# cvjena/ITAL

Hardware: AMD Instinct MI355X
Metric: MI-scored candidates/sec per fetch_unlabelled(k) round (higher is better)
Workload: dtype f64; 1 GPU; USPS-shaped synthetic 9298x256, k=4, perfect user, full 2^t enumeration, fetch_unlabelled + update per step; n=9298, d=256, k=4, parallelism=candidate rows sharded over 1 GPU(s), 1 record all-gather per greedy step

## Files before the change

ital_amd/_lib.py:

```python
import ctypes
import os

HERE = os.path.dirname(os.path.abspath(__file__))
LIB_PATH = os.environ.get("ITAL_HIP_LIB", os.path.join(HERE, "libital_hip.so"))

c_void_p, c_int, c_int64, c_double = ctypes.c_void_p, ctypes.c_int, ctypes.c_int64, ctypes.c_double

ITAL_MAX_T = 8
ITAL_REC_HEADER = 10
ITAL_JUMP_BITS = 48
ITAL_GENERIC_MAX_DIM = 20
ITAL_GENERIC_MAX_REL = 16
ITAL_GENERIC_MAX_CALLS = 1 << 22
ITAL_TOPK_MAX = 4096
ITAL_ROUND_MAX_CAND = 1 << 21


class ItalBatch(ctypes.Structure):
    _fields_ = [("kmax", c_int), ("ldx", c_int), ("ldw", c_int), ("bidx", c_void_p), ("bgpos", c_void_p),
                ("bsort", c_void_p), ("bmu", c_void_p), ("sig", c_void_p), ("XB", c_void_p), ("XBn", c_void_p),
                ("VB", c_void_p)]


class ItalLabelBatch(ctypes.Structure):
# ... 113 lines not shown
    "ital_score_generic_join": (c_int, [c_void_p]),
    "ital_ctx_create": (c_int, [c_int64, c_int, c_double, c_double, c_double, c_int, c_int, c_int, c_void_p, c_void_p]),
    "ital_ctx_destroy": (c_int, [c_void_p]),
    "ital_ctx_fit": (c_int, [c_void_p, c_void_p, c_int, c_void_p]),
    "ital_ctx_update": (c_int, [c_void_p, c_void_p, c_void_p, c_int, c_void_p]),
    "ital_ctx_fetch": (c_int, [c_void_p, c_int, c_void_p, c_void_p]),
    "ital_ctx_predict_stored": (c_int, [c_void_p, c_void_p, c_void_p, c_void_p]),
    "ital_ctx_local_rows": (c_int64, [c_void_p, c_void_p]),
    "ital_record_len": (c_int, [c_int, c_int, c_int]),
    "ital_round_workspace": (c_int64, [c_int, c_int64, c_int64]),
    "ital_sel_parts_len": (c_int64, [c_int, c_int64, c_int64]),
    "ital_mcmi_round": (c_int, [ctypes.POINTER(ItalMcmiRoundDesc), c_void_p]),
    "ital_gather_block": (c_int, [c_void_p, c_int64, c_int64, c_int64, c_void_p, c_void_p, c_int, c_void_p, c_int64, c_int,
                                  c_void_p, c_void_p, c_void_p, c_void_p, c_int64, c_void_p, c_void_p, c_void_p, c_void_p]),
    "ital_select_resolve": (c_int, [c_void_p, c_int, c_int, c_int, c_int, c_int, ItalBatch, c_void_p, c_void_p,
                                    c_void_p]),
}


class ItalCtxModel(ctypes.Structure):
    _fields_ = [("label_prob", c_double), ("mistake_prob", c_double), ("label_estimation", c_int),
                ("monte_carlo_num_rel", c_int), ("monte_carlo_num_fb", c_int), ("clip_cov", c_double)]


CTX_SIGNATURES = {
    "ital_ctx_set_model": (c_int, [c_void_p, ctypes.POINTER(ItalCtxModel)]),
    "ital_ctx_fetch_list": (c_int, [c_void_p, c_int, c_void_p, c_int64, c_void_p, c_int, c_void_p, c_void_p]),
    "ital_ctx_mcmi_fetch": (c_int, [c_void_p, c_int, c_void_p, c_int64, c_void_p, c_void_p]),
    "ital_ctx_top_results": (c_int, [c_void_p, c_int, c_void_p, c_void_p]),
    "ital_ctx_predict": (c_int, [c_void_p, c_void_p, c_int64, c_void_p, c_void_p, c_void_p]),
}


DENSE_SIGNATURES = {
    "ital_gram_rows": (c_int, [c_void_p, c_void_p, c_int, c_void_p, c_void_p, c_void_p, c_void_p, c_int, c_int, c_double,
                               c_double, c_double, c_void_p]),
    "ital_chol_batched": (c_int, [c_void_p, c_void_p, c_void_p, c_int, c_int, c_void_p, c_void_p, c_void_p]),
    "ital_chol_solve_batched": (c_int, [c_void_p, c_void_p, c_void_p, c_void_p, c_int, c_void_p, c_void_p]),
    "ital_kernel_matvec": (c_int, [c_void_p, c_void_p, c_int64, c_void_p, c_void_p, c_int64, c_int, c_void_p, c_int64, c_int,
                                   c_double, c_double, c_void_p, c_int64, c_void_p, c_int64, c_void_p]),
    "ital_kernel_matvec_workspace": (c_int64, [c_int64, c_int64]),
}


ADAPT_SIGNATURES = {
    "ital_chol_inv_diag": (c_int, [c_void_p, c_int, c_int64, c_void_p, c_void_p, c_int64, c_void_p, c_void_p]),
    "ital_chol_inv_diag_workspace": (c_int64, [c_int]),
    "ital_adapt_scores": (c_int, [c_void_p, c_void_p, c_void_p, c_int64, c_double, c_void_p, c_void_p, c_void_p]),
    "ital_adapt_error": (c_int, [c_void_p, c_int64, c_void_p, c_int, c_int64, c_void_p, c_void_p, c_double, c_void_p,
                                 c_void_p, c_void_p]),
}


class ItalHipError(RuntimeError):
    pass


def load(path=LIB_PATH):
    if not os.path.exists(path):
        raise ImportError(
            f"{path} not found: build it with `python -m ital_amd.build` (hipcc, gfx950). "
            "ital_amd has no CPU fallback.")
    try:
        import torch
    except ImportError:
        pass
    lib = ctypes.CDLL(path)
    for name, (res, args) in list(SIGNATURES.items()) + list(CTX_SIGNATURES.items()) + list(DENSE_SIGNATURES.items()) + \
            list(ADAPT_SIGNATURES.items()):
        fn = getattr(lib, name)
        fn.restype = res
        fn.argtypes = args
    return lib


_lib = None


def lib():
    global _lib
    if _lib is None:
        _lib = load()
    return _lib


def check(rc):
    if rc != 0:
        raise ItalHipError(f"libital_hip: error {rc}: {lib().ital_last_error().decode()}")


def legacy_normals(n_skip, n_out, threads=1):
    import numpy as np
    n_skip, n_out = int(n_skip), int(n_out)
    state = np.random.get_state(legacy=True)
    if state[0] != "MT19937":
        if n_skip:
            np.random.standard_normal(n_skip)
        return np.random.standard_normal(n_out)
    st = ItalNpLegacyState()
    key = np.ascontiguousarray(state[1], dtype=np.uint32)
    ctypes.memmove(st.key, key.ctypes.data, 624 * 4)
    st.pos, st.has_gauss, st.gauss = int(state[2]), int(state[3]), float(state[4])
    out = np.empty(n_out, dtype=np.float64)
    check(lib().ital_np_legacy_normals(ctypes.byref(st), n_skip, out.ctypes.data, n_out, int(threads)))
    np.random.set_state(("MT19937", np.frombuffer(st.key, dtype=np.uint32).copy(), int(st.pos), int(st.has_gauss),
                         float(st.gauss)))
    return out
```

ital_amd/build.py:

```python
import os
import subprocess
import sys
from concurrent.futures import ThreadPoolExecutor

HERE = os.path.dirname(os.path.abspath(__file__))
CSRC = os.path.join(HERE, "csrc")
INCLUDE = os.path.join(os.path.dirname(HERE), "include")
LIB = os.path.join(HERE, "libital_hip.so")
SOURCES = ["api.hip", "rbf.hip", "chol.hip", "score.hip", "select.hip", "mcmi.hip", "score_generic.hip", "gen_pipeline.hip", "topk.hip", "exchange.hip", "round.hip", "ctx.hip", "dense.hip", "adapt.hip",
           "mvn_stream.cpp", "np_legacy.cpp"]
HIPCC = os.environ.get("HIPCC", "/opt/rocm/bin/hipcc")
EXTRA = os.environ.get("ITAL_HIPCC_EXTRA", "").split()
HOST_EXTRA = os.environ.get("ITAL_HOST_EXTRA", "").split()
LINK_EXTRA = os.environ.get("ITAL_LINK_EXTRA", "").split()
LIB = os.environ.get("ITAL_HIP_LIB_OUT", LIB)
FLAGS = EXTRA + ["--offload-arch=gfx950", "-O3", "-std=c++17", "-fPIC", "-fno-gpu-rdc",
         "-I", INCLUDE, "-I", CSRC, "-Wall", "-Wno-unused-function"]
HOST_FLAGS = ["-O3", "-std=c++17", "-fPIC", "-ffp-contract=off", "-I", INCLUDE, "-I", CSRC, "-Wall"]


def _newer(target, deps):
    if not os.path.exists(target):
        return True
    t = os.path.getmtime(target)
    return any(os.path.getmtime(d) > t for d in deps)


def build(force=False, verbose=False):
    headers = [os.path.join(CSRC, f) for f in os.listdir(CSRC) if f.endswith(".h")] + \
              [os.path.join(INCLUDE, "ital_hip.h"), os.path.join(INCLUDE, "ital_ctx.h"), os.path.join(INCLUDE, "ital_dense.h"),
               os.path.join(INCLUDE, "ital_adapt.h")]
    objdir = os.environ.get("ITAL_OBJ_DIR", os.path.join(HERE, "_obj"))
    os.makedirs(objdir, exist_ok=True)
    jobs = []
    objs = []
    for src in SOURCES:
        s = os.path.join(CSRC, src)
        o = os.path.join(objdir, os.path.splitext(src)[0] + ".o")
        objs.append(o)
        if force or _newer(o, [s] + headers):
            jobs.append([HIPCC] + (FLAGS if src.endswith(".hip") else HOST_FLAGS + HOST_EXTRA) + ["-c", s, "-o", o])

    def run(cmd):
        if verbose:
            print(" ".join(cmd), flush=True)
        subprocess.check_call(cmd)

    if jobs:
        with ThreadPoolExecutor(max_workers=4) as ex:
            list(ex.map(run, jobs))
    if jobs or force or _newer(LIB, objs):
        run([HIPCC, "--offload-arch=gfx950", "-shared", "-fPIC", "-o", LIB] + LINK_EXTRA + objs + ["-ldl", "-lpthread"])
    return LIB


if __name__ == "__main__":
    print(build(force="--force" in sys.argv, verbose=True))
```

ital_amd/csrc/score.hip:

```cpp
#include <hip/hip_runtime.h>
#include <stdint.h>

#include <type_traits>

#include "device_math.h"
#include "ital_hip.h"
#include "ital_internal.h"
#include "qmc_common.h"
#include "qmc_exact.h"
#include "qmc_seed.h"
#include "qmc_share.h"
#include "select_common.h"

#ifndef ITAL_QMC_HOTK
#define ITAL_QMC_HOTK 1
#endif
#ifndef ITAL_QMC_MAIN_NH
#define ITAL_QMC_MAIN_NH(T) ((T) == 6 || (T) == 8 ? 2 : 3)
#endif
#ifndef ITAL_QMC_WAVES
#define ITAL_QMC_WAVES(T) ((T) <= 4 || (T) == 6 || (T) == 8 ? 4 : 3)
#endif
#ifndef ITAL_QMC_MAIN_PS
#define ITAL_QMC_MAIN_PS(T) ((T) >= 7)
#endif
#ifndef ITAL_QMC_MAIN_KE6
#define ITAL_QMC_MAIN_KE6(T) ((T) == 8)
#endif
#ifndef ITAL_QMC_MAIN_KEN
#define ITAL_QMC_MAIN_KEN(T) ((T) == 7 ? 2 : -1)
#endif
#ifndef ITAL_QMC_MAIN_KE
#define ITAL_QMC_MAIN_KE(T) 1
#endif
#ifndef ITAL_QMC_MAIN_KS
#define ITAL_QMC_MAIN_KS(T) 0
#endif
#ifndef ITAL_QMC_MAIN_CFL
#define ITAL_QMC_MAIN_CFL(T) ((T) >= 7)
#endif

#ifndef ITAL_QMC_SHARE_LAST
#define ITAL_QMC_SHARE_LAST 1
#endif
#ifndef ITAL_QMC_SHARE_RECS
#define ITAL_QMC_SHARE_RECS 4
#endif
#ifndef ITAL_QMC_SHARE_VCF
#define ITAL_QMC_SHARE_VCF 3
#endif

namespace ital {

struct ScoreArgs {
    int t;
    int64_t n_cand;
    const int32_t* cand;
    const uint8_t* alive;
    const double* mu;
    const double* s2;
    const double* C;
    int64_t ldc;
    int64_t row_offset;
    int64_t pos_offset;
    const int64_t* gpos;
    ital_batch b;
    double noise, eps;
    int label_mode;
    double* mi;
    int seed[6];
    const long long* jump;
    const long long* jumppat;
    const double* vk;
    int* status;
    SelectTail sel;
};

__device__ __forceinline__ double log_eps(double p, double eps) { return log(p + eps); }

__device__ __forceinline__ void mi_accumulate(double& mi, double pr, double pu, double eps, int mode) {
    double cur = log_eps(pu, eps) - log_eps(pr, eps);
    if (mode == 1) {
        if (cur > mi) mi = cur;
    } else if (mode == 2) {
        if (mi == 0 || cur < mi) mi = cur;
    } else {
        mi += cur * pr;
    }
}

__global__ __launch_bounds__(256) void score_t1_kernel(ScoreArgs a) {
    const int64_t p = (int64_t)blockIdx.x * blockDim.x + threadIdx.x;
    const bool valid = p < a.n_cand && a.alive[p];
    double mi = 0.0;
    if (valid) {
        const int row = a.cand[p];
        const double mu = a.mu[row];
        const double su = a.s2[row];
        const double sc = fmax(0.0, su);
        const double p_irr = norm_cdf0(mu, sqrt(sc));
        const double w = 1.0 / (su + a.noise);
        const double g = su * w;
// ... 43 lines not shown
            const double c00 = a.noise * g00, c11 = a.noise * g11, c01 = a.noise * g01;
            const double t0 = sqrt(c00), t1 = sqrt(c11);
            double h = -u0 / t0, k = -u1 / t1;
            const double rho = c01 / (t0 * t1);
            const int64_t gi = a.row_offset + row;
            if (gi < a.b.bidx[0]) val = bvn_orthant(k, h, rel1, rel0, rho);
            else val = bvn_orthant(h, k, rel0, rel1, rho);
        }
    }
    vals[updated ? 1 : 0][pair] = val;
    __syncthreads();
    Best c = {0.0, -1, 0};
    if (threadIdx.x < 32) {
        const int64_t pc = (int64_t)blockIdx.x * 32 + threadIdx.x;
        if (pc < a.n_cand && a.alive[pc]) {
            double mi = 0.0;
#pragma unroll
            for (int q = 0; q < 4; q++) mi_accumulate(mi, vals[0][4 * threadIdx.x + q], vals[1][4 * threadIdx.x + q], a.eps, a.label_mode);
            a.mi[pc] = mi;
            c.val = mi;
            c.pos = a.gpos ? a.gpos[pc] : a.pos_offset + pc;
            c.loc = pc;
        }
    }
    if (a.sel.enabled) {
        c = block_best(c, 0);
        select_tail(a.sel, c, blockIdx.x, gridDim.x, true, gridDim.x);
    }
}

template <int T>
struct Qmc {
    static constexpr int NDIM = T - 1;
    static constexpr int NP = NDIM < 10 ? NDIM : 10;
    static constexpr int PRIME = P_TAB[NP - 1];
    static constexpr int NCOV = T * (T + 1) / 2;
    static constexpr int NCOR = T * (T - 1) / 2;
    static constexpr int NPAT = 1 << T;
    static constexpr int NCALLS = 2 << T;
    static constexpr int LAT = 8 * NDIM * 2;
    static constexpr int LATP = 5 * NDIM;
    static constexpr int R_LIM = NCOR, R_META = NCOR + T, R_LAT = NCOR + T + 1;
    static constexpr int REC = R_LAT + LATP;
    static constexpr int SLAB_RAW = NCOV + 2 * T + NDIM;
    static constexpr int SLAB = SLAB_RAW | 1;
    static constexpr int PREP_THREADS = T <= 6 ? 256 : 128;
    static constexpr int NH = ITAL_QMC_MAIN_NH(T);
    static constexpr int TAILQ = 128 * NH;
    static constexpr bool PS = ITAL_QMC_MAIN_PS(T), CFL = PS && ITAL_QMC_MAIN_CFL(T);
    static constexpr bool SHARE = ITAL_QMC_SHARE_LAST && ITAL_QMC_HOTK && ITAL_QMC_FLIP && !PS &&
                                  QmcRounds<T, NH>::NCL == 1 && ITAL_QMC_SHARE_RECS * QmcRounds<T, NH>::REST <= 64 &&
                                  NPAT % ITAL_QMC_SHARE_RECS == 0;
    static constexpr int RPW = SHARE ? ITAL_QMC_SHARE_RECS : 1;
    static constexpr int WAVE_DOUBLES = LAT + TAILQ + (CFL ? NCOR + T : 0) + (SHARE ? 64 + 2 * RPW + 6 : 0);
    typedef typename std::conditional<(CFL && ITAL_QMC_MAIN_KS(T)), HotKS,
                typename std::conditional<(ITAL_QMC_MAIN_KEN(T) >= 0), HotKEn<(ITAL_QMC_MAIN_KEN(T) >= 0 ? ITAL_QMC_MAIN_KEN(T) : 0)>,
                typename std::conditional<(ITAL_QMC_MAIN_KE6(T)), HotKE6,
                    typename std::conditional<(ITAL_QMC_MAIN_KE(T)), HotKE, HotK>::type>::type>::type>::type Coef;
    static constexpr int64_t CAND_DOUBLES = (int64_t)NPAT * (REC + 1) + 3;
};
constexpr long long META_EVAL = 1, META_PRIOR_ONE = 2, META_POST_ONE = 4;
constexpr long long META_EXACT = 8;

template <int T>
__device__ void rcswp(int p, int q, double* cov, double* lim, unsigned& infi) {
    double tmp = lim[p]; lim[p] = lim[q]; lim[q] = tmp;
    unsigned bp = (infi >> p) & 1u, bq = (infi >> q) & 1u;
    infi = (infi & ~((1u << p) | (1u << q))) | (bq << p) | (bp << q);
    tmp = cov[pidx(p, p)]; cov[pidx(p, p)] = cov[pidx(q, q)]; cov[pidx(q, q)] = tmp;
    for (int j = 0; j < p; j++) { tmp = cov[pidx(p, j)]; cov[pidx(p, j)] = cov[pidx(q, j)]; cov[pidx(q, j)] = tmp; }
    for (int i = p + 1; i < q; i++) { tmp = cov[pidx(i, p)]; cov[pidx(i, p)] = cov[pidx(q, i)]; cov[pidx(q, i)] = tmp; }
    for (int i = q + 1; i < T; i++) { tmp = cov[pidx(i, p)]; cov[pidx(i, p)] = cov[pidx(i, q)]; cov[pidx(i, q)] = tmp; }
}

template <int T>
__device__ bool covsrt(double* cov, double* lim, double* y, unsigned& infi) {
    const double SQTWPI = 2.506628274631001, EPS = 1e-10;
    bool ok = true;
    for (int i = 0; i < T; i++) {
        double dmin = 0, emin = 1, zmin = 0, cvdiag = 0;
        int jmin = i;
        for (int j = i; j < T; j++) {
            const double cjj = cov[pidx(j, j)];
            if (cjj > EPS) {
                const double sumsq = sqrt_pos(cjj);
                double sum = 0;
                for (int k = 0; k < i; k++) sum += cov[pidx(j, k)] * y[k];
                const double z = fast_div(lim[j] - sum, sumsq);
                const double ph = mvn_phi(z);
                const bool lower = (infi >> j) & 1u;
                const double d = lower ? ph : 0.0;
                const double e = lower ? 1.0 : fmax(ph, 0.0);
                if (emin + d >= e + dmin) { jmin = j; zmin = z; dmin = d; emin = e; cvdiag = sumsq; }
            }
        }
        if (jmin > i) rcswp<T>(i, jmin, cov, lim, infi);
        cov[pidx(i, i)] = cvdiag;
        if (cvdiag > 0) {
            const double rdiag = fast_div(1.0, cvdiag);
            for (int l = i + 1; l < T; l++) {
                cov[pidx(l, i)] = cov[pidx(l, i)] * rdiag;
                for (int j = i + 1; j <= l; j++) cov[pidx(l, j)] -= cov[pidx(l, i)] * cov[pidx(j, i)];
            }
            const bool lower = (infi >> i) & 1u;
            if (emin > dmin + EPS) {
                const double dens = -exp_neg(-zmin * zmin / 2) * (1.0 / SQTWPI);
                const double yl = lower ? dens : 0.0, yu = lower ? 0.0 : dens;
// ... 134 lines not shown
            atomicOr(a.status, 2);
        } else {
            bool sat1 = true, sat0 = false;
            for (int v = 0; v < T; v++) {
                double bound = 0;
                for (int j = 0; j < v; j++) bound += fabs(cov[pidx(v, j)]) * 9.0;
                const bool lower = (infi >> v) & 1u;
                if (lower) {
                    if (!(lim[v] + bound < -37.0)) sat1 = false;
                    if (lim[v] - bound > 37.0) sat0 = true;
                } else {
                    if (!(lim[v] - bound > 37.0)) sat1 = false;
                    if (lim[v] + bound < -37.0) sat0 = true;
                }
            }
            if (sat0) verdict = 4;
            else if (sat1) verdict = 2;
            else evaluate = true;
        }
    }
    if (verdict == 2) meta |= META_PRIOR_ONE;
    if (evaluate) {
        meta |= META_EVAL | ((long long)infi << 8);
        const unsigned fl = ITAL_QMC_FLIP ? infi : 0u;
        for (int v = 1; v < T; v++)
            for (int j = 0; j < v; j++)
                rec[v * (v - 1) / 2 + j] = (((fl >> v) ^ (fl >> j)) & 1u) ? -cov[pidx(v, j)] : cov[pidx(v, j)];
        for (int v = 0; v < T; v++) rec[Q::R_LIM + v] = ((fl >> v) & 1u) ? -lim[v] : lim[v];
        const int* sp = seeds + i * 6;
        MrgState sti = {sp[0], sp[1], sp[2], sp[3], sp[4], sp[5]};
        mrg_apply(sti, a.jumppat + (int64_t)r * 18);
        MrgStateF st = mrg_to_f(sti);
        for (int j = 0; j < Q::NDIM; j++) gen[j] = (double)j;
        unsigned int* shifts = reinterpret_cast<unsigned int*>(rec + Q::R_LAT);
        unsigned char* perm = reinterpret_cast<unsigned char*>(rec + Q::R_LAT + 4 * Q::NDIM);
        for (int sft = 0; sft < 8; sft++) {
            for (int j = 1; j <= Q::NDIM - 1; j++) {
                const double u = mrg_next_f(st);
                const int jp = (int)(j + u * (Q::NDIM + 1 - j));
                const double xt = gen[j - 1];
                gen[j - 1] = gen[jp - 1];
                gen[jp - 1] = xt;
            }
            for (int j = 0; j < Q::NDIM; j++) perm[sft * Q::NDIM + j] = (unsigned char)gen[j];
            for (int j = 0; j < Q::NDIM; j++) shifts[sft * Q::NDIM + j] = (unsigned int)mrg_next_z(st);
        }
    }
    rec[Q::R_META] = __longlong_as_double(meta);
}

template <int T>
__device__ __forceinline__ void qmc_main_shared(const uint8_t* __restrict__ alive, int64_t slab_lo, int64_t slab_n,
                                                const double* __restrict__ recs, const double* __restrict__ vk, double eps,
                                                int label_mode, double* __restrict__ terms) {
    using Q = Qmc<T>;
    using R = QmcRounds<T, Q::NH>;
    extern __shared__ double lds_all[];
    const int lane = threadIdx.x & 63;
    const int wid = __builtin_amdgcn_readfirstlane(threadIdx.x >> 6);
    const int64_t item0 = ((int64_t)blockIdx.x * 4 + wid) * Q::RPW;
    const int64_t i = item0 >> T;
    if (i >= slab_n) return;
    if (!alive[slab_lo + i]) return;
    double* lat = lds_all + (size_t)wid * Q::WAVE_DOUBLES;
    double* tailq = lat + Q::LAT;
    int first = -1;
    for (int j = Q::RPW - 1; j >= 0; j--)
        if (__double_as_longlong(uniform_f64(recs[(item0 + j) * Q::REC + Q::R_META])) & META_EVAL) first = j;
    double* lastv = tailq + Q::TAILQ;
    typename Q::Coef kk;
    kk.load();
    if (first >= 0) {
        const int j_own = lane >> 4;
        bool dead = j_own >= Q::RPW;
        if (!dead) dead = !(__double_as_longlong(recs[(item0 + j_own) * Q::REC + Q::R_META]) & META_EVAL);
        const double* rec = recs + (item0 + (dead ? first : j_own)) * Q::REC;
        const unsigned flips = (unsigned)(__double_as_longlong(rec[Q::R_META]) >> 8) & ((1u << T) - 1u);
        double cf[Q::NCOR > 0 ? Q::NCOR : 1], lm[T], xx[Q::NDIM > 0 ? Q::NDIM : 1];
#pragma unroll
        for (int q = 0; q < Q::NCOR; q++) cf[q] = rec[q];
#pragma unroll
        for (int q = 0; q < T; q++) lm[q] = rec[Q::R_LIM + q];
        const unsigned int* shifts = reinterpret_cast<const unsigned int*>(rec + Q::R_LAT);
        const unsigned char* perm = reinterpret_cast<const unsigned char*>(rec + Q::R_LAT + 4 * Q::NDIM);
        const int it = R::FULL * 64 * Q::NH + ((lane & 15) >> 1);
        const int sft = it / Q::PRIME;
        const int k = it - sft * Q::PRIME + 1;
#pragma unroll
        for (int j = 0; j < Q::NDIM; j++) {
            const int q = sft * Q::NDIM + j;
            const double gen = vk[perm[q]];
            const double shf = (double)shifts[q] * MRG_INVMP1 + (((flips >> (q % Q::NDIM)) & 1u) ? 0.5 : 0.0);
            const double v = k * gen + shf;
            const double fr = v - floor(v);
            const double x = fabs(2 * fr - 1);
            xx[j] = (lane & 1) ? 1 - x : x;
        }
        double w0;
        lastv[lane] = eval_chain_lanes<T, typename Q::Coef>(xx, dead, cf, lm, flips, tailq, lane, kk, w0);
        if ((lane & 15) == 0 && j_own < Q::RPW) lastv[64 + Q::RPW + j_own] = w0;
    }
    double* keep = lastv + 64 + 2 * Q::RPW;
    if (lane == 0) {
        keep[0] = __longlong_as_double((long long)recs);
        keep[1] = __longlong_as_double((long long)vk);
        keep[2] = __longlong_as_double((long long)terms);
        keep[3] = eps;
        keep[4] = __longlong_as_double((long long)label_mode);
        keep[5] = __longlong_as_double(item0);
    }
    __builtin_amdgcn_fence(__ATOMIC_RELEASE, "wavefront");
    __builtin_amdgcn_wave_barrier();
    __builtin_amdgcn_fence(__ATOMIC_ACQUIRE, "wavefront");
    int jv = 0;
    for (;;) {
        int ln = lane;
        __asm__ volatile("" : "+v"(ln), "+v"(jv));
        const int j = __builtin_amdgcn_readfirstlane(jv);
        if (j >= Q::RPW) break;
        const double* rec = reinterpret_cast<const double*>(__double_as_longlong(uniform_f64(keep[0]))) +
                            (__double_as_longlong(uniform_f64(keep[5])) + j) * Q::REC;
        const long long meta = __double_as_longlong(uniform_f64(rec[Q::R_META]));
        double pr = (meta & META_PRIOR_ONE) ? 1.0 : 0.0;
        if (meta & META_EVAL) {
            const unsigned flips = (unsigned)(meta >> 8) & ((1u << T) - 1u);
            __builtin_amdgcn_fence(__ATOMIC_RELEASE, "wavefront");
            __builtin_amdgcn_wave_barrier();
            {
                const double* vk_j = reinterpret_cast<const double*>(__double_as_longlong(uniform_f64(keep[1])));
                const unsigned int* shifts = reinterpret_cast<const unsigned int*>(rec + Q::R_LAT);
                const unsigned char* perm = reinterpret_cast<const unsigned char*>(rec + Q::R_LAT + 4 * Q::NDIM);
                for (int q = ln; q < 8 * Q::NDIM; q += 64) {
                    lat[q] = vk_j[perm[q]];
                    lat[8 * Q::NDIM + q] = (double)shifts[q] * MRG_INVMP1 + (((flips >> (q % Q::NDIM)) & 1u) ? 0.5 : 0.0);
                }
            }
            double cf[Q::NCOR > 0 ? Q::NCOR : 1], lm[T];
#pragma unroll
            for (int q = 0; q < Q::NCOR; q++) cf[q] = q >= Q::NCOR - ITAL_QMC_SHARE_VCF ? rec[q] : uniform_f64(rec[q]);
#pragma unroll
            for (int q = 0; q < T; q++) lm[q] = uniform_f64(rec[Q::R_LIM + q]);
            __builtin_amdgcn_fence(__ATOMIC_RELEASE, "wavefront");
            __builtin_amdgcn_wave_barrier();
            __builtin_amdgcn_fence(__ATOMIC_ACQUIRE, "wavefront");
            const double w0 = lastv[64 + Q::RPW + j];
            const double part = qmc_lane_sum_full<T, typename Q::Coef, Q::NH>(lat, w0, cf, lm, flips, tailq, ln, kk);
            __asm__ volatile("" : "+v"(jv));
            const int j2 = __builtin_amdgcn_readfirstlane(jv);
            const double acc = part + (ln < 16 ? lastv[16 * j2 + ln] : 0.0);
            pr = wave_sum(acc) / (16.0 * Q::PRIME);
#ifndef ITAL_NO_EXACT_FLAG
            if ((pr > 1.0 - EXACT_BAND || pr < EXACT_BAND) && ln == 0 && __double_as_longlong(keep[4]) != 0) {
                double* rm = reinterpret_cast<double*>(__double_as_longlong(keep[0])) + (__double_as_longlong(keep[5]) + j2) * Q::REC + Q::R_META;
                *rm = __longlong_as_double(__double_as_longlong(*rm) | META_EXACT);
            }
#endif
        }
        __asm__ volatile("" : "+v"(jv));
        if (ln == 0) lastv[64 + __builtin_amdgcn_readfirstlane(jv)] = pr;
        jv = jv + 1;
    }
    __builtin_amdgcn_fence(__ATOMIC_RELEASE, "wavefront");
    __builtin_amdgcn_wave_barrier();
    __builtin_amdgcn_fence(__ATOMIC_ACQUIRE, "wavefront");
    if (lane < Q::RPW) {
        const double* recs_k = reinterpret_cast<const double*>(__double_as_longlong(keep[0]));
        double* terms_k = reinterpret_cast<double*>(__double_as_longlong(keep[2]));
        const long long item_l = __double_as_longlong(keep[5]) + lane;
        const double eps_k = keep[3];
        const double pr_l = lastv[64 + lane];
        const long long meta_l = __double_as_longlong(recs_k[item_l * Q::REC + Q::R_META]);
        const double pu = (meta_l & META_POST_ONE) ? 1.0 : 0.0;
        const double cur = log_eps(pu, eps_k) - log_eps(pr_l, eps_k);
        terms_k[item_l] = __double_as_longlong(keep[4]) == 0 ? cur * pr_l : cur;
    }
}

template <int T>
__global__ __launch_bounds__(256) __attribute__((amdgpu_waves_per_eu(ITAL_QMC_WAVES(T), ITAL_QMC_WAVES(T)))) void qmc_main_kernel(
    const uint8_t* __restrict__ alive, int64_t slab_lo, int64_t slab_n, const double* __restrict__ recs,
    const double* __restrict__ vk, double eps, int label_mode, double* __restrict__ terms) {
    using Q = Qmc<T>;
    if constexpr (Q::SHARE) {
        qmc_main_shared<T>(alive, slab_lo, slab_n, recs, vk, eps, label_mode, terms);
        return;
    }
    extern __shared__ double lds_all[];
    const int lane = threadIdx.x & 63;
    const int wid = __builtin_amdgcn_readfirstlane(threadIdx.x >> 6);
    const int64_t item = (int64_t)blockIdx.x * 4 + wid;
    const int64_t i = item >> T;
    if (i >= slab_n) return;
    if (!alive[slab_lo + i]) return;
    const double* rec = recs + item * Q::REC;
    const long long meta = __double_as_longlong(uniform_f64(rec[Q::R_META]));
    double pr = (meta & META_PRIOR_ONE) ? 1.0 : 0.0;
    if (meta & META_EVAL) {
        double* lat = lds_all + (size_t)wid * Q::WAVE_DOUBLES;
        double* tailq = lat + Q::LAT;
        const unsigned flips = ITAL_QMC_FLIP ? (unsigned)(meta >> 8) & ((1u << T) - 1u) : 0u;
        {
            const unsigned int* shifts = reinterpret_cast<const unsigned int*>(rec + Q::R_LAT);
            const unsigned char* perm = reinterpret_cast<const unsigned char*>(rec + Q::R_LAT + 4 * Q::NDIM);
            for (int q = lane; q < 8 * Q::NDIM; q += 64) {
                lat[q] = vk[perm[q]];
                lat[8 * Q::NDIM + q] = (double)shifts[q] * MRG_INVMP1 + (((flips >> (q % Q::NDIM)) & 1u) ? 0.5 : 0.0);
            }
        }
        double cf[Q::NCOR > 0 ? Q::NCOR : 1], lm[T];
        double* slab = tailq + Q::TAILQ;
        if (Q::CFL) {
            for (int q = lane; q < Q::NCOR + T; q += 64) slab[q] = rec[q];
        } else {
#pragma unroll
            for (int q = 0; q < Q::NCOR; q++) cf[q] = uniform_f64(rec[q]);
#pragma unroll
            for (int q = 0; q < T; q++) lm[q] = uniform_f64(rec[Q::R_LIM + q]);
        }
        const unsigned infi = (unsigned)(meta >> 8) & ((1u << T) - 1u);
        __builtin_amdgcn_fence(__ATOMIC_RELEASE, "wavefront");
        __builtin_amdgcn_wave_barrier();
        __builtin_amdgcn_fence(__ATOMIC_ACQUIRE, "wavefront");
#if ITAL_QMC_HOTK
        typename Q::Coef kk;
        kk.load();
        constexpr bool FL = ITAL_QMC_FLIP != 0;
        const double acc = Q::PS ? qmc_lane_sum_ps<T, typename Q::Coef, Q::NH, Q::CFL, FL>(lat, cf, lm, slab, infi, tailq, lane, kk)
                                 : qmc_lane_sum<T, typename Q::Coef, Q::NH, FL>(lat, cf, lm, infi, tailq, lane, kk);
#else
        const double acc = qmc_lane_sum<T, LitK, Q::NH, ITAL_QMC_FLIP != 0>(lat, cf, lm, infi, tailq, lane);
#endif
        pr = wave_sum(acc) / (16.0 * Q::PRIME);
#ifndef ITAL_NO_EXACT_FLAG
        if (label_mode != 0 && (pr > 1.0 - EXACT_BAND || pr < EXACT_BAND) && lane == 0)
            const_cast<double*>(rec)[Q::R_META] = __longlong_as_double(meta | META_EXACT);
#endif
    }
    if (lane == 0) {
        const double pu = (meta & META_POST_ONE) ? 1.0 : 0.0;
        const double cur = log_eps(pu, eps) - log_eps(pr, eps);
        terms[item] = label_mode == 0 ? cur * pr : cur;
    }
}
// ... 11 lines not shown
    const double* rec = recs + item * Q::REC;
    const long long meta = __double_as_longlong(uniform_f64(rec[Q::R_META]));
    if (!(meta & META_EXACT)) return;
    double* slab = lds_all;
    double* lat = slab + Q::NCOV + T;
    double* tailq = lat + Q::LAT;
    double* vals = tailq + 128;
    const unsigned infi = (unsigned)(meta >> 8) & ((1u << T) - 1u);
    const unsigned fl = ITAL_QMC_FLIP ? infi : 0u;
    for (int q = lane; q < Q::NCOV; q += 64) {
        int row = 0;
        while ((row + 1) * (row + 2) / 2 <= q) row++;
        const int col = q - row * (row + 1) / 2;
        double v = 0.0;
        if (col < row) {
            v = rec[row * (row - 1) / 2 + col];
            if (((fl >> row) ^ (fl >> col)) & 1u) v = -v;
        }
        slab[q] = v;
    }
    for (int q = lane; q < T; q += 64) slab[Q::NCOV + q] = ((fl >> q) & 1u) ? -rec[Q::R_LIM + q] : rec[Q::R_LIM + q];
    {
        const unsigned int* shifts = reinterpret_cast<const unsigned int*>(rec + Q::R_LAT);
        const unsigned char* perm = reinterpret_cast<const unsigned char*>(rec + Q::R_LAT + 4 * Q::NDIM);
        for (int q = lane; q < 8 * Q::NDIM; q += 64) {
            lat[q] = vk[perm[q]];
            lat[8 * Q::NDIM + q] = (double)shifts[q] * MRG_INVMP1;
        }
    }
    __builtin_amdgcn_fence(__ATOMIC_RELEASE, "wavefront");
    __builtin_amdgcn_wave_barrier();
    __builtin_amdgcn_fence(__ATOMIC_ACQUIRE, "wavefront");
    qmc_point_values<T>(T, slab, infi, (1u << T) - 1u, lat, lane, tailq, vals);
    __builtin_amdgcn_fence(__ATOMIC_RELEASE, "wavefront");
    __builtin_amdgcn_wave_barrier();
    __builtin_amdgcn_fence(__ATOMIC_ACQUIRE, "wavefront");
    const double pr = mvkbrv_serial(Q::PRIME, vals, lane);
    if (lane == 0) {
        const double pu = (meta & META_POST_ONE) ? 1.0 : 0.0;
        const double cur = log_eps(pu, eps) - log_eps(pr, eps);
        terms[item] = label_mode == 0 ? cur * pr : cur;
    }
}

__global__ __launch_bounds__(256) void qmc_combine_kernel(const double* __restrict__ terms, const uint8_t* __restrict__ alive,
                                                          int64_t slab_lo, int64_t slab_n, int npat, int label_mode,
                                                          double* __restrict__ mi, int64_t pos_offset,
                                                          const int64_t* __restrict__ gpos, SelectTail sel, int part0,
                                                          int nparts, int finishing) {
    const int64_t i = (int64_t)blockIdx.x * blockDim.x + threadIdx.x;
    const bool valid = i < slab_n && alive[slab_lo + i];
    double s = 0.0;
    if (valid) {
        for (int r = 0; r < npat; r++) {
            const double cur = terms[i * npat + r];
            if (label_mode == 1) { if (cur > s) s = cur; }
            else if (label_mode == 2) { if (s == 0 || cur < s) s = cur; }
            else s += cur;
        }
        mi[slab_lo + i] = s;
    }
    if (sel.enabled) {
        const int64_t p = slab_lo + i;
        Best c = {s, valid ? (gpos ? gpos[p] : pos_offset + p) : -1, p};
        c = block_best(c, 0);
        select_tail(sel, c, part0 + blockIdx.x, nparts, finishing != 0, gridDim.x);
    }
}

template <int T>
static int launch_qmc(const ScoreArgs& a, double* work, int64_t work_doubles, int64_t sel_parts_len, hipEvent_t ev0, hipEvent_t ev1,
                      hipStream_t stream, bool seeds_ready, SeedArgs* seeds_only) {
    using Q = Qmc<T>;
    int64_t slab = work_doubles / Q::CAND_DOUBLES;
    if (slab < 1) return ital_fail(-12, "ital_score_step: workspace smaller than one candidate (see ital_score_workspace)");
    if (slab > a.n_cand) slab = a.n_cand;
    const size_t lds_main = (size_t)4 * Q::WAVE_DOUBLES * sizeof(double);
    const size_t lds_prep = (size_t)Q::PREP_THREADS * Q::SLAB * sizeof(double);
    static ItalLdsFlags lds_flags;
    if (lds_prep > 48 * 1024) {
        const int rc = ital_raise_lds_limit(reinterpret_cast<const void*>(&qmc_prep_kernel<T>), (int)lds_prep, lds_flags,
                                            "ital_score_step");
        if (rc) return rc;
    }
    double* recs = work;
    double* terms = recs + slab * Q::NPAT * Q::REC;
    int* seeds = reinterpret_cast<int*>(terms + slab * Q::NPAT);
    if (seeds_only) {
        if (slab < a.n_cand) return 1;
        *seeds_only = seed_args(a, Q::NCALLS, 0, a.n_cand, seeds);
        return 0;
    }
    int nparts = 0, part0 = 0;
    for (int64_t lo = 0; lo < a.n_cand; lo += slab) nparts += (int)(((a.n_cand - lo < slab ? a.n_cand - lo : slab) + 255) / 256);
    if (a.sel.enabled && 3 * (int64_t)nparts > sel_parts_len)
        return ital_fail(-22, "ital_score_step: sel_parts too small for the blocks of this step");
    for (int64_t lo = 0; lo < a.n_cand; lo += slab) {
        const int64_t n = a.n_cand - lo < slab ? a.n_cand - lo : slab;
        if (!(seeds_ready && slab >= a.n_cand))
            ITAL_LAUNCH(qmc_seed_kernel, dim3((unsigned)((n + 255) / 256)), dim3(256), 0, stream, seed_args(a, Q::NCALLS, lo, n, seeds));
        ITAL_LAUNCH(qmc_prep_kernel<T>, dim3((unsigned)((n + Q::PREP_THREADS - 1) / Q::PREP_THREADS), Q::NPAT),
                           dim3(Q::PREP_THREADS), lds_prep, stream, a, lo, n, seeds, recs);
        if (ev0 && lo == 0) (void)hipEventRecord(ev0, stream);
        ITAL_LAUNCH(qmc_main_kernel<T>, dim3((unsigned)((n * Q::NPAT + 4 * Q::RPW - 1) / (4 * Q::RPW))), dim3(256), lds_main, stream, a.alive, lo,
                           n, recs, a.vk, a.eps, a.label_mode, terms);
        if (ev1 && lo + n >= a.n_cand) (void)hipEventRecord(ev1, stream);
        if (a.label_mode != 0) {
            const size_t lds_x = (size_t)(Q::NCOV + T + Q::LAT + 128 + 16 * Q::PRIME) * sizeof(double);
            static ItalLdsFlags lds_xflags;
            if (lds_x > 48 * 1024) {
                const int rc = ital_raise_lds_limit(reinterpret_cast<const void*>(&qmc_exact_kernel<T>), (int)lds_x, lds_xflags, "ital_score_step");
                if (rc) return rc;
            }
            ITAL_LAUNCH(qmc_exact_kernel<T>, dim3((unsigned)(n * Q::NPAT)), dim3(64), lds_x, stream, a.alive, lo, n, recs, a.vk, a.eps,
                        a.label_mode, terms);
        }
        ITAL_LAUNCH(qmc_combine_kernel, dim3((unsigned)((n + 255) / 256)), dim3(256), 0, stream, terms, a.alive, lo, n,
                    Q::NPAT, a.label_mode, a.mi, a.pos_offset, a.gpos, a.sel, part0, nparts, lo + n >= a.n_cand ? 1 : 0);
        part0 += (int)((n + 255) / 256);
        int rc = ital_check_launch("ital_score_step(qmc)");
        if (rc) return rc;
    }
    return 0;
}

template <int T>
static int64_t qmc_cand_doubles() { return Qmc<T>::CAND_DOUBLES; }

static int64_t cand_doubles(int t) {
    switch (t) {
        case 3: return qmc_cand_doubles<3>();
        case 4: return qmc_cand_doubles<4>();
        case 5: return qmc_cand_doubles<5>();
        case 6: return qmc_cand_doubles<6>();
        case 7: return qmc_cand_doubles<7>();
        case 8: return qmc_cand_doubles<8>();
    }
    return 0;
}

}

using namespace ital;

extern "C" int64_t ital_score_workspace(int t, int64_t n_cand) {
    if (t < 3 || t > ITAL_MAX_T || n_cand <= 0) return 0;
    return cand_doubles(t) * n_cand;
}

extern "C" int ital_record_len(int ldx, int ldw, int kmax) {
    if (ldx < 0 || ldw < 0 || kmax < 0) return 0;
    return ITAL_REC_HEADER + ldx + ldw + kmax;
}

extern "C" int64_t ital_round_workspace(int k, int64_t n_cand, int64_t cap_doubles) {
    if (k > ITAL_MAX_T) k = ITAL_MAX_T;
    const int64_t one_slab = ital_score_workspace(k, n_cand > 0 ? n_cand : 1);
    if (one_slab == 0) return 0;
    int64_t cap = cap_doubles > 0 ? cap_doubles : one_slab;
    const int64_t least = ital_score_workspace(k, 1);
    if (cap < least) cap = least;
    return one_slab < cap ? one_slab : cap;
}

extern "C" int64_t ital_sel_parts_len(int k, int64_t n_cand, int64_t work_doubles) {
    if (n_cand < 0) n_cand = 0;
    if (k > ITAL_MAX_T) k = ITAL_MAX_T;
    int64_t slabs = 0;
    if (k >= 3 && n_cand > 0) {
        const int64_t per = ital_score_workspace(k, 1);
        const int64_t fit = work_doubles / per;
        slabs = fit >= n_cand ? 1 : (fit < 1 ? n_cand : (n_cand + fit - 1) / fit);
    }
    return 3 * (n_cand / 32 + 64 + slabs);
}

int ital_score_step_internal(const ital_score_desc* d, hipStream_t stream, bool seeds_ready, ital::SeedArgs* seeds_only) {
    if (!d) return ital_fail(-22, "ital_score_step: null descriptor");
    if (seeds_only && (d->n_cand <= 0 || d->t < 3 || d->t > ITAL_MAX_T || !d->work || !d->jump)) return 1;
    if (d->n_cand <= 0) return 0;
    if (d->t < 1 || d->t > ITAL_MAX_T) return ital_fail(-22, "ital_score_step: batch dimension outside 1..ITAL_MAX_T");
    if (d->t > d->batch.kmax) return ital_fail(-22, "ital_score_step: t exceeds the batch capacity");
    ScoreArgs a = {};
    a.t = d->t; a.n_cand = d->n_cand; a.cand = d->cand; a.alive = d->alive; a.mu = d->mu; a.s2 = d->s2; a.C = d->C;
    a.ldc = d->ldc; a.row_offset = d->row_offset; a.pos_offset = d->pos_offset; a.gpos = d->gpos; a.b = d->batch;
    a.noise = d->noise; a.eps = d->eps; a.label_mode = d->label_mode; a.mi = d->mi; a.jump = d->jump;
    a.jumppat = d->jumppat; a.vk = d->vk; a.status = d->status;
    for (int i = 0; i < 6; i++) a.seed[i] = d->seed[i];
    if (d->sel_record) {
        if (!d->sel_parts || !d->sel_counter || !d->sel_X || !d->sel_xnorm || (d->sel_m > 0 && !d->sel_V))
            return ital_fail(-22, "ital_score_step: fused selection needs sel_parts, sel_counter, sel_X, sel_xnorm, sel_V");
        if (d->sel_m > d->sel_ldw || d->sel_ldx != d->batch.ldx || d->sel_ldw != d->batch.ldw)
            return ital_fail(-22, "ital_score_step: fused selection: batch layout mismatch");
        a.sel.rec = {d->cand, d->pos_offset, d->gpos, d->row_offset, d->sel_rank, 0, 0, d->mu, d->s2, d->sel_X, d->sel_xnorm,
                     d->sel_ldx, d->sel_V, d->sel_ldv, d->sel_m, d->sel_ldw, d->C, d->ldc, d->t - 1, d->batch.kmax, nullptr,
                     d->sel_record, d->status};
// ... 38 lines not shown
```

Baseline: 15.74 million candidates/s.

## Plan QMC main-kernel work items with a single-record tail and ballot meta loads

Adds an item plan for the shared-record QMC main kernel that splits work into four-record items plus an optional tail of single-record items, with the tail size set from resident wave occupancy or a runtime override. It also replaces the per-record serial META loads with one per-lane load and a ballot, and unrolls the combine kernel's reduction over patterns in chunks of 16. The default tail is zero, so the plan reproduces the old four-record grid, and the main live changes are the ballot-based metadata read and the unrolled combine loop. It adds an occupancy query on first use and a per-wave skip offset to handle partial items.

```diff
diff --git a/include/ital_plan.h b/include/ital_plan.h
--- /dev/null
+++ b/include/ital_plan.h
@@ -0,0 +1,17 @@
+#ifndef ITAL_PLAN_H
+#define ITAL_PLAN_H
+
+#include "ital_hip.h"
+
+#ifdef __cplusplus
+extern "C" {
+#endif
+
+int ital_qmc_item_plan(int t, int64_t n_cand, int64_t resident_waves, int64_t tail_records, int64_t* n4, int64_t* n1);
+
+int64_t ital_qmc_plan_tail(int64_t tail_records);
+
+#ifdef __cplusplus
+}
+#endif
+#endif
diff --git a/ital_amd/_lib.py b/ital_amd/_lib.py
--- a/ital_amd/_lib.py
+++ b/ital_amd/_lib.py
@@ -189,6 +189,12 @@
 }
 
 
+PLAN_SIGNATURES = {
+    "ital_qmc_item_plan": (c_int, [c_int, c_int64, c_int64, c_int64, ctypes.POINTER(c_int64), ctypes.POINTER(c_int64)]),
+    "ital_qmc_plan_tail": (c_int64, [c_int64]),
+}
+
+
 class ItalHipError(RuntimeError):
     pass
 
@@ -204,7 +210,7 @@
         pass
     lib = ctypes.CDLL(path)
     for name, (res, args) in list(SIGNATURES.items()) + list(CTX_SIGNATURES.items()) + list(DENSE_SIGNATURES.items()) + \
-            list(ADAPT_SIGNATURES.items()):
+            list(ADAPT_SIGNATURES.items()) + list(PLAN_SIGNATURES.items()):
         fn = getattr(lib, name)
         fn.restype = res
         fn.argtypes = args
diff --git a/ital_amd/build.py b/ital_amd/build.py
--- a/ital_amd/build.py
+++ b/ital_amd/build.py
@@ -29,7 +29,7 @@
 def build(force=False, verbose=False):
     headers = [os.path.join(CSRC, f) for f in os.listdir(CSRC) if f.endswith(".h")] + \
               [os.path.join(INCLUDE, "ital_hip.h"), os.path.join(INCLUDE, "ital_ctx.h"), os.path.join(INCLUDE, "ital_dense.h"),
-               os.path.join(INCLUDE, "ital_adapt.h")]
+               os.path.join(INCLUDE, "ital_adapt.h"), os.path.join(INCLUDE, "ital_plan.h")]
     objdir = os.environ.get("ITAL_OBJ_DIR", os.path.join(HERE, "_obj"))
     os.makedirs(objdir, exist_ok=True)
     jobs = []
diff --git a/ital_amd/csrc/score.hip b/ital_amd/csrc/score.hip
--- a/ital_amd/csrc/score.hip
+++ b/ital_amd/csrc/score.hip
@@ -1,11 +1,13 @@
 #include <hip/hip_runtime.h>
 #include <stdint.h>
 
+#include <atomic>
 #include <type_traits>
 
 #include "device_math.h"
 #include "ital_hip.h"
 #include "ital_internal.h"
+#include "ital_plan.h"
 #include "qmc_common.h"
 #include "qmc_exact.h"
 #include "qmc_seed.h"
@@ -48,6 +50,13 @@
 #endif
 #ifndef ITAL_QMC_SHARE_VCF
 #define ITAL_QMC_SHARE_VCF 3
+#endif
+
+#ifndef ITAL_QMC_TAIL_PER_SLOT
+#define ITAL_QMC_TAIL_PER_SLOT 0
+#endif
+#ifndef ITAL_QMC_MAIN_WPB
+#define ITAL_QMC_MAIN_WPB(T) 4
 #endif
 
 namespace ital {
@@ -197,7 +206,8 @@
                                   QmcRounds<T, NH>::NCL == 1 && ITAL_QMC_SHARE_RECS * QmcRounds<T, NH>::REST <= 64 &&
                                   NPAT % ITAL_QMC_SHARE_RECS == 0;
     static constexpr int RPW = SHARE ? ITAL_QMC_SHARE_RECS : 1;
-    static constexpr int WAVE_DOUBLES = LAT + TAILQ + (CFL ? NCOR + T : 0) + (SHARE ? 64 + 2 * RPW + 6 : 0);
+    static constexpr int WAVE_DOUBLES = LAT + TAILQ + (CFL ? NCOR + T : 0) + (SHARE ? 64 + 2 * RPW + 7 : 0);
+    static constexpr int WPB = ITAL_QMC_MAIN_WPB(T);
     typedef typename std::conditional<(CFL && ITAL_QMC_MAIN_KS(T)), HotKS,
                 typename std::conditional<(ITAL_QMC_MAIN_KEN(T) >= 0), HotKEn<(ITAL_QMC_MAIN_KEN(T) >= 0 ? ITAL_QMC_MAIN_KEN(T) : 0)>,
                 typename std::conditional<(ITAL_QMC_MAIN_KE6(T)), HotKE6,
@@ -438,28 +448,31 @@
 template <int T>
 __device__ __forceinline__ void qmc_main_shared(const uint8_t* __restrict__ alive, int64_t slab_lo, int64_t slab_n,
                                                 const double* __restrict__ recs, const double* __restrict__ vk, double eps,
-                                                int label_mode, double* __restrict__ terms) {
+                                                int label_mode, double* __restrict__ terms, int64_t n4, int64_t n1) {
     using Q = Qmc<T>;
     using R = QmcRounds<T, Q::NH>;
     extern __shared__ double lds_all[];
     const int lane = threadIdx.x & 63;
     const int wid = __builtin_amdgcn_readfirstlane(threadIdx.x >> 6);
-    const int64_t item0 = ((int64_t)blockIdx.x * 4 + wid) * Q::RPW;
-    const int64_t i = item0 >> T;
+    const int64_t w = (int64_t)blockIdx.x * Q::WPB + wid;
+    if (w >= n4 + n1) return;
+    const int skip = w < n4 ? 0 : Q::RPW - 1;
+    const int64_t item0 = (w < n4 ? w * Q::RPW : n4 * Q::RPW + (w - n4)) - skip;
+    const int64_t i = (item0 + skip) >> T;
     if (i >= slab_n) return;
     if (!alive[slab_lo + i]) return;
     double* lat = lds_all + (size_t)wid * Q::WAVE_DOUBLES;
     double* tailq = lat + Q::LAT;
-    int first = -1;
-    for (int j = Q::RPW - 1; j >= 0; j--)
-        if (__double_as_longlong(uniform_f64(recs[(item0 + j) * Q::REC + Q::R_META])) & META_EVAL) first = j;
+    long long meta_own = 0;
+    if (lane >= skip && lane < Q::RPW) meta_own = __double_as_longlong(recs[(item0 + lane) * Q::REC + Q::R_META]);
+    const unsigned evals = (unsigned)__ballot((meta_own & META_EVAL) != 0);
+    const int first = evals ? __builtin_ctz(evals) : -1;
     double* lastv = tailq + Q::TAILQ;
     typename Q::Coef kk;
     kk.load();
     if (first >= 0) {
         const int j_own = lane >> 4;
-        bool dead = j_own >= Q::RPW;
-        if (!dead) dead = !(__double_as_longlong(recs[(item0 + j_own) * Q::REC + Q::R_META]) & META_EVAL);
+        const bool dead = !((evals >> j_own) & 1u);
         const double* rec = recs + (item0 + (dead ? first : j_own)) * Q::REC;
         const unsigned flips = (unsigned)(__double_as_longlong(rec[Q::R_META]) >> 8) & ((1u << T) - 1u);
         double cf[Q::NCOR > 0 ? Q::NCOR : 1], lm[T], xx[Q::NDIM > 0 ? Q::NDIM : 1];
@@ -494,11 +507,12 @@
         keep[3] = eps;
         keep[4] = __longlong_as_double((long long)label_mode);
         keep[5] = __longlong_as_double(item0);
+        keep[6] = __longlong_as_double((long long)skip);
     }
     __builtin_amdgcn_fence(__ATOMIC_RELEASE, "wavefront");
     __builtin_amdgcn_wave_barrier();
     __builtin_amdgcn_fence(__ATOMIC_ACQUIRE, "wavefront");
-    int jv = 0;
+    int jv = skip;
     for (;;) {
         int ln = lane;
         __asm__ volatile("" : "+v"(ln), "+v"(jv));
@@ -549,7 +563,7 @@
     __builtin_amdgcn_fence(__ATOMIC_RELEASE, "wavefront");
     __builtin_amdgcn_wave_barrier();
     __builtin_amdgcn_fence(__ATOMIC_ACQUIRE, "wavefront");
-    if (lane < Q::RPW) {
+    if (lane >= (int)__double_as_longlong(keep[6]) && lane < Q::RPW) {
         const double* recs_k = reinterpret_cast<const double*>(__double_as_longlong(keep[0]));
         double* terms_k = reinterpret_cast<double*>(__double_as_longlong(keep[2]));
         const long long item_l = __double_as_longlong(keep[5]) + lane;
@@ -563,18 +577,18 @@
 }
 
 template <int T>
-__global__ __launch_bounds__(256) __attribute__((amdgpu_waves_per_eu(ITAL_QMC_WAVES(T), ITAL_QMC_WAVES(T)))) void qmc_main_kernel(
+__global__ __launch_bounds__(64 * ITAL_QMC_MAIN_WPB(T)) __attribute__((amdgpu_waves_per_eu(ITAL_QMC_WAVES(T), ITAL_QMC_WAVES(T)))) void qmc_main_kernel(
     const uint8_t* __restrict__ alive, int64_t slab_lo, int64_t slab_n, const double* __restrict__ recs,
-    const double* __restrict__ vk, double eps, int label_mode, double* __restrict__ terms) {
+    const double* __restrict__ vk, double eps, int label_mode, double* __restrict__ terms, int64_t n4, int64_t n1) {
     using Q = Qmc<T>;
     if constexpr (Q::SHARE) {
-        qmc_main_shared<T>(alive, slab_lo, slab_n, recs, vk, eps, label_mode, terms);
+        qmc_main_shared<T>(alive, slab_lo, slab_n, recs, vk, eps, label_mode, terms, n4, n1);
         return;
     }
     extern __shared__ double lds_all[];
     const int lane = threadIdx.x & 63;
     const int wid = __builtin_amdgcn_readfirstlane(threadIdx.x >> 6);
-    const int64_t item = (int64_t)blockIdx.x * 4 + wid;
+    const int64_t item = (int64_t)blockIdx.x * Q::WPB + wid;
     const int64_t i = item >> T;
     if (i >= slab_n) return;
     if (!alive[slab_lo + i]) return;
@@ -692,11 +706,22 @@
     const bool valid = i < slab_n && alive[slab_lo + i];
     double s = 0.0;
     if (valid) {
-        for (int r = 0; r < npat; r++) {
-            const double cur = terms[i * npat + r];
-            if (label_mode == 1) { if (cur > s) s = cur; }
-            else if (label_mode == 2) { if (s == 0 || cur < s) s = cur; }
-            else s += cur;
+        const double* tp = terms + i * npat;
+        for (int r0 = 0; r0 < npat; r0 += 16) {
+            double cur[16];
+#pragma unroll
+            for (int q = 0; q < 16; q++) cur[q] = tp[r0 + q < npat ? r0 + q : 0];
+            const int m = npat - r0;
+            if (label_mode == 1) {
+#pragma unroll
+                for (int q = 0; q < 16; q++) if (q < m && cur[q] > s) s = cur[q];
+            } else if (label_mode == 2) {
+#pragma unroll
+                for (int q = 0; q < 16; q++) if (q < m && (s == 0 || cur[q] < s)) s = cur[q];
+            } else {
+#pragma unroll
+                for (int q = 0; q < 16; q++) if (q < m) s += cur[q];
+            }
         }
         mi[slab_lo + i] = s;
     }
@@ -706,6 +731,65 @@
         c = block_best(c, 0);
         select_tail(sel, c, part0 + blockIdx.x, nparts, finishing != 0, gridDim.x);
     }
+}
+
+static std::atomic<int64_t> g_plan_tail{-1};
+
+static int share_recs(int t) {
+    switch (t) {
+        case 3: return Qmc<3>::RPW;
+        case 4: return Qmc<4>::RPW;
+        case 5: return Qmc<5>::RPW;
+        case 6: return Qmc<6>::RPW;
+        case 7: return Qmc<7>::RPW;
+        case 8: return Qmc<8>::RPW;
+    }
+    return 1;
+}
+
+static int item_plan(int t, int64_t n_cand, int64_t resident_waves, int64_t tail_records, int64_t* n4, int64_t* n1) {
+    if (t < 3 || t > ITAL_MAX_T) return ital_fail(-22, "ital_qmc_item_plan: batch dimension outside 3..ITAL_MAX_T");
+    if (n_cand < 1 || n_cand > ((int64_t)1 << 40)) return ital_fail(-22, "ital_qmc_item_plan: n_cand outside 1..2^40");
+    if (resident_waves < 0) return ital_fail(-22, "ital_qmc_item_plan: negative resident_waves");
+    if (tail_records < -1) return ital_fail(-22, "ital_qmc_item_plan: tail_records below -1");
+    if (!n4 || !n1) return ital_fail(-22, "ital_qmc_item_plan: null result pointer");
+    const int64_t recs = n_cand << t;
+    const int rpw = share_recs(t);
+    if (rpw == 1) {
+        *n4 = 0;
+        *n1 = recs;
+        return 0;
+    }
+    int64_t tail = tail_records;
+    if (tail < 0)
+        tail = ITAL_QMC_TAIL_PER_SLOT == 0 ? 0 : (resident_waves >= recs ? recs : (int64_t)ITAL_QMC_TAIL_PER_SLOT * resident_waves);
+    tail = tail >= recs ? recs : (tail + rpw - 1) / rpw * rpw;
+    *n1 = tail;
+    *n4 = (recs - tail) / rpw;
+    return 0;
+}
+
+template <int T>
+static int plan_items(int64_t n, int64_t resident, int64_t* n4, int64_t* n1) {
+    static_assert(!Qmc<T>::SHARE || Qmc<T>::RPW == 4, "the plan's long items are four records");
+    return item_plan(T, n, resident, g_plan_tail.load(std::memory_order_relaxed), n4, n1);
+}
+
+struct ResidentWaves { std::atomic<int64_t> waves[16]; ResidentWaves() { for (auto& w : waves) w.store(-1); } };
+static int64_t resident_waves(ResidentWaves& cache, const void* kernel, int wpb, size_t lds) {
+    int dev = 0;
+    if (hipGetDevice(&dev) != hipSuccess || dev < 0 || dev >= 16) { (void)hipGetLastError(); return 0; }
+    int64_t w = cache.waves[dev].load(std::memory_order_relaxed);
+    if (w >= 0) return w;
+    int blocks = 0, cus = 0;
+    if (hipOccupancyMaxActiveBlocksPerMultiprocessor(&blocks, kernel, 64 * wpb, lds) != hipSuccess ||
+        hipDeviceGetAttribute(&cus, hipDeviceAttributeMultiprocessorCount, dev) != hipSuccess || blocks < 0 || cus < 0) {
+        (void)hipGetLastError();
+        blocks = cus = 0;
+    }
+    w = (int64_t)blocks * wpb * cus;
+    cache.waves[dev].store(w, std::memory_order_relaxed);
+    return w;
 }
 
 template <int T>
@@ -715,7 +799,7 @@
     int64_t slab = work_doubles / Q::CAND_DOUBLES;
     if (slab < 1) return ital_fail(-12, "ital_score_step: workspace smaller than one candidate (see ital_score_workspace)");
     if (slab > a.n_cand) slab = a.n_cand;
-    const size_t lds_main = (size_t)4 * Q::WAVE_DOUBLES * sizeof(double);
+    const size_t lds_main = (size_t)Q::WPB * Q::WAVE_DOUBLES * sizeof(double);
     const size_t lds_prep = (size_t)Q::PREP_THREADS * Q::SLAB * sizeof(double);
     static ItalLdsFlags lds_flags;
     if (lds_prep > 48 * 1024) {
@@ -730,6 +814,11 @@
         if (slab < a.n_cand) return 1;
         *seeds_only = seed_args(a, Q::NCALLS, 0, a.n_cand, seeds);
         return 0;
+    }
+    int64_t resident = 0;
+    if (Q::SHARE) {
+        static ResidentWaves cache;
+        resident = resident_waves(cache, reinterpret_cast<const void*>(&qmc_main_kernel<T>), Q::WPB, lds_main);
     }
     int nparts = 0, part0 = 0;
     for (int64_t lo = 0; lo < a.n_cand; lo += slab) nparts += (int)(((a.n_cand - lo < slab ? a.n_cand - lo : slab) + 255) / 256);
@@ -742,8 +831,13 @@
         ITAL_LAUNCH(qmc_prep_kernel<T>, dim3((unsigned)((n + Q::PREP_THREADS - 1) / Q::PREP_THREADS), Q::NPAT),
                            dim3(Q::PREP_THREADS), lds_prep, stream, a, lo, n, seeds, recs);
         if (ev0 && lo == 0) (void)hipEventRecord(ev0, stream);
-        ITAL_LAUNCH(qmc_main_kernel<T>, dim3((unsigned)((n * Q::NPAT + 4 * Q::RPW - 1) / (4 * Q::RPW))), dim3(256), lds_main, stream, a.alive, lo,
-                           n, recs, a.vk, a.eps, a.label_mode, terms);
+        int64_t n4 = 0, n1 = n * Q::NPAT;
+        if (Q::SHARE) {
+            const int rc = plan_items<T>(n, resident, &n4, &n1);
+            if (rc) return rc;
+        }
+        ITAL_LAUNCH(qmc_main_kernel<T>, dim3((unsigned)((n4 + n1 + Q::WPB - 1) / Q::WPB)), dim3(64 * Q::WPB), lds_main, stream, a.alive, lo,
+                           n, recs, a.vk, a.eps, a.label_mode, terms, n4, n1);
         if (ev1 && lo + n >= a.n_cand) (void)hipEventRecord(ev1, stream);
         if (a.label_mode != 0) {
             const size_t lds_x = (size_t)(Q::NCOV + T + Q::LAT + 128 + 16 * Q::PRIME) * sizeof(double);
@@ -782,6 +876,15 @@
 }
 
 using namespace ital;
+
+extern "C" int ital_qmc_item_plan(int t, int64_t n_cand, int64_t resident_waves, int64_t tail_records, int64_t* n4, int64_t* n1) {
+    return item_plan(t, n_cand, resident_waves, tail_records, n4, n1);
+}
+
+extern "C" int64_t ital_qmc_plan_tail(int64_t tail_records) {
+    if (tail_records < -1) return ital_fail(-22, "ital_qmc_plan_tail: tail_records below -1");
+    return g_plan_tail.exchange(tail_records);
+}
 
 extern "C" int64_t ital_score_workspace(int t, int64_t n_cand) {
     if (t < 3 || t > ITAL_MAX_T || n_cand <= 0) return 0;
```

After: 15.72 million candidates/s. About the same (-0.1%).
